# iscc/iscc-search

Hardware: AMD Instinct MI355X
Metric: queries/sec (+ roofline of the dominant kernel), 64-bit Hamming k=10 over 100M codes, exact top-k (higher is better)
Workload: dtype fp4 (e2m1 0/1 x +-1 products, f32 accumulation: exact integers)

## Files before the change

### iscc_search_amd/csrc/batch.hip.h

```cpp

void launch_scan(int W, bool mask, int tq, int mode, dim3 grid, hipStream_t st, const isk::ScanParams& p) {
    auto with_tq = [&](auto&& f) { if (tq == 8) f(isk::int_c<8>{}); else f(isk::int_c<16>{}); };
    if (W == 1 && !mask) {
        isk::with_mode(mode, [&](auto m) { with_tq([&](auto t) {
            if constexpr (decltype(m)::value != isk::MODE_SELF) hipLaunchKernelGGL((isk::scan_adapt_kernel<decltype(t)::value, decltype(m)::value>), grid, dim3(isk::BLOCK), 0, st, p);
        }); });
        return;
    }
    isk::with_words(W, [&](auto w) {
        auto masked = [&](auto mk) { with_tq([&](auto t) { isk::with_mode(mode, [&](auto m) {
            constexpr int WORDS = decltype(w)::value, MODE = decltype(m)::value;
            constexpr bool MASK = decltype(mk)::value;
            if constexpr (MODE != isk::MODE_SELF && (WORDS > 1 || MASK)) hipLaunchKernelGGL((isk::scan_kernel<WORDS, MASK, decltype(t)::value, MODE>), grid, dim3(isk::BLOCK), 0, st, p);
        }); }); };
        if (mask) masked(std::true_type{}); else masked(std::false_type{});
    });
}
int tile_rows_for(int W) { return W == 1 ? isk::tile_rows<1>() : W == 2 ? isk::tile_rows<2>() : W == 3 ? isk::tile_rows<3>() : isk::tile_rows<4>(); }

constexpr uint64_t CACHE_RESIDENT_BYTES = 128ull << 20;
uint32_t scan_grid_x(H* h, int W, uint64_t rows, uint32_t groups = 1, bool sample = false) {
    const uint64_t tiles = rows / (uint64_t)tile_rows_for(W);
    uint64_t maxb = (uint64_t)h->cus * BLOCKS_PER_CU;
    if (sample || rows * 8 * (uint64_t)W <= CACHE_RESIDENT_BYTES)
// ... 57 lines not shown
    isk::Record* d_out;
    uint32_t* d_out_cnt;
    uint32_t* d_out_rows = nullptr;
    uint32_t* d_out_kth = nullptr;
    int tq = 8;
    int radius = -1;
    double radius_ratio = -1.0;
    bool ratio_starts_self = false;
    size_t pq_off = 0;
    uint32_t* d_flags = nullptr;
    const uint32_t* h_flags = nullptr;
    uint32_t nq_pad = 0, groups = 0, cap = 0, P = 0;
    size_t sel_lds = 0;
    bool multi = false;
    bool mark_overflow = false;
    bool allow_self = true, used_self = false;
    int self_hint = -1;
    bool used_hint = false;
    bool on_matrix_cores = false;
    std::vector<Job> jobs;

    Batch(H* h_, Table& t_, uint32_t nq_, uint32_t qbytes_, uint32_t k_, isk::Record* out, uint32_t* out_cnt)
        : h(h_), t(t_), nq(nq_), qbytes(qbytes_), k(k_), d_out(out), d_out_cnt(out_cnt) {}

    int ratio_bits(int bits) const { return std::min(bits, (int)std::floor(radius_ratio * bits + 1e-9)); }
    int ratio_bits(const Job& j) const { return ratio_bits(8 * (int)j.pbytes); }
    int job_radius(const Job& j) const {
        if (radius >= 0) return radius;
        if (radius_ratio >= 0 && !ratio_starts_self) return ratio_bits(j);
        return -1;
    }
    struct Ctx { isk::ScanParams sp; isk::SelectParams sl; };
    Ctx make_ctx(size_t ji) const {
        const Job& j = jobs[ji];
        Segment& s = *j.seg;
        Ctx c{};
        set_cols(c.sp.col, s, j.W);
        c.sp.queries = h->d_queries.p; c.sp.bias = h->d_bias.p; c.sp.cnt = h->d_cnt.p; c.sp.cand = h->d_cand.p;
        c.sp.ghist = h->d_ghist.p; c.sp.cap = cap; c.sp.k = k; c.sp.fold_tau = FOLD_TAU; c.sp.nq_pad = nq_pad;
        c.sp.mask_lo = (uint32_t)j.mask_last; c.sp.mask_hi = (uint32_t)(j.mask_last >> 32);
        c.sp.thr_live = h->d_thr.p;
        c.sp.refresh_steps = SELF_REFRESH_STEPS;
        c.sl.cnt = h->d_cnt.p; c.sl.cand = h->d_cand.p; c.sl.cap = cap; c.sl.keys = s.keys;
        c.sl.rank = h->d_rank + (t.metric == ISCCSEARCH_METRIC_NPHD ? j.pbytes * 257 : 0);
        c.sl.out = multi ? h->d_lists.p + ji * (size_t)nq * k : d_out;
        c.sl.out_count = multi ? h->d_listcnt.p + ji * (size_t)nq : d_out_cnt;
        c.sl.overflow = d_flags + ji * (size_t)nq_pad;
        c.sl.k = k; c.sl.P = P; c.sl.prefix_bits = j.pbytes * 8; c.sl.q_base = 0;
        c.sl.overflow_count = mark_overflow ? isk::COUNT_OVERFLOW : 0;
        c.sl.out_rows = multi ? nullptr : d_out_rows;
        c.sl.out_kth = multi ? nullptr : d_out_kth;
        return c;
    }
    struct Run { const Job& j; Ctx c; int radius; bool hist_live = false; };

    template <typename F>
    void with_record_form(const isk::SelectParams& sl, F&& f) const {
        auto keyed = [&](auto rows) { isk::with_key_words(t.key_words, [&](auto kw) { f(kw, rows); }); };
        if (sl.out_rows) keyed(std::true_type{}); else keyed(std::false_type{});
    }
    template <int NT>
    void launch_select_nt(const isk::SelectParams& sl, uint32_t blocks) const {
        with_record_form(sl, [&](auto kw, auto rows) { hipLaunchKernelGGL((isk::select_kernel<decltype(kw)::value, decltype(rows)::value, NT>), dim3(blocks), dim3(NT), sel_lds, h->stream, sl); });
    }
    void launch_select(const isk::SelectParams& sl, uint32_t blocks) const {
        const uint64_t wide_from = (uint64_t)h->opt.select_wide_from;
        const bool wide = sl.P >= wide_from && (sl.P >= 2 * wide_from || blocks <= (uint32_t)h->cus / 2);
        if (wide) launch_select_nt<1024>(sl, blocks);
        else launch_select_nt<isk::BLOCK>(sl, blocks);
    }
    bool tiny(const Job& j) const { return j.seg->n <= (uint64_t)h->opt.tiny_rows && j.seg->n <= cap && j.seg->n < (uint64_t)h->opt.mfma_min_rows; }
    template <int NT>
    void launch_tiny_nt(const isk::TinyParams& tp, const isk::SelectParams& sl, const isk::InlineQueries& iq) const {
        with_record_form(sl, [&](auto kw, auto rows) { hipLaunchKernelGGL((isk::tiny_search_kernel<decltype(kw)::value, decltype(rows)::value, NT>), dim3(nq), dim3(NT), sel_lds, h->stream, tp, sl, iq); });
    }
    size_t flag_words() const { return jobs.size() * (size_t)nq_pad; }

    bool use_mfma(const Job& j, uint64_t rows) const {
        const bool from_nine = j.pack || j.seg->n <= MFMA_FEW_ROWS;
        const uint32_t min_queries = (uint32_t)h->opt.mfma_min_queries;
        return h->opt.mfma && (on_matrix_cores || nq_pad >= (from_nine ? std::min(min_queries, MFMA_PACK_MIN_QUERIES) : min_queries)) && rows >= (uint64_t)h->opt.mfma_min_rows;
    }
    bool single_pass(const Job& j) const { return allow_self && h->opt.self_tighten && use_mfma(j, j.seg->n); }
    enum class Path { tiny, radius, single, levels };
    Path path(const Job& j) const {
        if (tiny(j)) return Path::tiny;
        if (job_radius(j) >= 0) return Path::radius;
        return single_pass(j) ? Path::single : Path::levels;
    }
    bool pack3(const Job& j) const { return j.pack && h->opt.mfma_pack3 && isk::mfma_pack3_fits(isk::mfma_groups_per_chunk((int)j.W, nq_pad, j.pack)); }
    bool pack3_pass(const Job& j) const { return use_mfma(j, j.seg->n) && pack3(j); }
    int scan(const Job& j, const isk::ScanParams& sp, int mode, bool sample) {
        const uint64_t rows = sp.n_rows - sp.row_begin;
        if (use_mfma(j, rows) || mode == isk::MODE_SELF) {
            const uint32_t g = isk::mfma_groups_per_chunk((int)j.W, nq_pad, j.pack);
            const uint32_t chunks = (nq_pad + g * 32 - 1) / (g * 32);
            const bool pack3 = this->pack3(j);
            const uint64_t rps = isk::mfma_rows_per_wave_step((int)j.W, j.pack, pack3);
            const uint64_t steps = (rows + rps - 1) / rps;
            const uint64_t wpb = isk::mfma_waves_per_block();
            const uint64_t bx = std::max<uint64_t>(1, std::min<uint64_t>((steps + wpb - 1) / wpb, std::max<uint32_t>(1, (uint32_t)h->cus * isk::mfma_blocks_per_cu((int)j.W, g, j.pack) / chunks)));
            const int e = isk::launch_mfma_scan((int)j.W, mode, j.pack, (uint32_t)bx, g, h->stream, sp, pack3);
            if (e) return fail(-EIO, "mfma scan: chunk of %u query groups does not fit the LDS budget (%s)", g, hipGetErrorString((hipError_t)e));
            h->stats.mfma_launches += 1;
            if (j.pack) h->stats.mfma_pack_launches += 1;
            h->stats.mfma_pair_words += rows * (uint64_t)nq * j.W;
            return 0;
// ... 5 lines not shown
    }

    void plan(const uint64_t* hq) {
        jobs.clear();
        tq = (int)h->opt.queries_per_pass;
        if (tq == 8 && nq > 8 && nq <= 16) tq = 16;
        nq_pad = (nq + tq - 1) / tq * tq;
        groups = nq_pad / tq;
        for (uint32_t b = 1; b <= ISCCSEARCH_MAX_BYTES; ++b) {
            Segment& s = t.seg[b];
            if (!s.n) continue;
            Job j;
            j.seg = &s;
            j.pbytes = t.metric == ISCCSEARCH_METRIC_NPHD ? std::min(b, qbytes) : b;
            j.W = (j.pbytes + 7) / 8;
            j.mask = (j.pbytes & 7) != 0;
            j.mask_last = mask_for(j.pbytes);
            j.pack = h->opt.mfma_pack && j.W == 1;
            if (j.pack && j.pbytes == 8)
                for (uint32_t q = 0; q < nq && j.pack; ++q) j.pack = hq[(size_t)q * t.max_words] != 0;
            jobs.push_back(j);
        }
    }
    int reserve() {
        cap = std::max<uint32_t>((uint32_t)h->opt.candidate_cap, 16 * k);
        if (h->opt.self_tighten && h->opt.mfma && radius < 0 && radius_ratio < 0) cap = std::max<uint32_t>(cap, 64 * k);
        multi = jobs.size() > 1;
        P = next_pow2(std::max<uint32_t>(std::max<uint32_t>(k, 1024), std::min<uint32_t>(4 * k, 4096)));
        sel_lds = (((size_t)P * 4 + 15) & ~(size_t)15) + (size_t)P * 8 * t.key_words + (d_out_rows ? (size_t)P * 4 : 0);
        int rc;
        if ((rc = h->d_queries.ensure((size_t)nq_pad * 4))) return rc;
        if ((rc = h->d_bias.ensure(nq_pad))) return rc;
        if ((rc = h->d_thr.ensure(nq_pad))) return rc;
        if ((rc = h->d_cnt.ensure((size_t)nq_pad * isk::CNT_STRIDE))) return rc;
        if ((rc = h->d_ghist.ensure((size_t)nq_pad * isk::HB))) return rc;
        if (!d_flags) {
            if ((rc = h->d_overflow.ensure(flag_words()))) return rc;
            d_flags = h->d_overflow.p;
        }
        if ((rc = h->d_cand.ensure((size_t)nq_pad * cap))) return rc;
        if (multi) {
            if ((rc = h->d_lists.ensure(jobs.size() * (size_t)nq * k))) return rc;
            if ((rc = h->d_listcnt.ensure(jobs.size() * (size_t)nq))) return rc;
        }
        return 0;
    }
    const uint64_t* staged() const { return h->p_queries.p + pq_off; }
    bool all_tiny() const {
        for (const Job& j : jobs) if (!tiny(j)) return false;
        return true;
    }
    bool inline_queries() const { return !all_tiny() && radius >= 0 && nq_pad <= isk::INLINE_QUERIES && jobs.size() == 1; }
    bool tiny_inline() const { return all_tiny() && nq_pad <= isk::INLINE_QUERIES; }
    int stage(const uint64_t* hq) {
        int rc;
        if ((rc = wait_staged(h))) return rc;
        if ((rc = h->p_queries.ensure(pq_off + (size_t)nq_pad * 4))) return rc;
        uint64_t* const pq = h->p_queries.p + pq_off;
        memset(pq, 0, (size_t)nq_pad * 4 * 8);
        for (uint32_t q = 0; q < nq; ++q)
            for (int w = 0; w < t.max_words; ++w) pq[(size_t)q * 4 + w] = hq[(size_t)q * t.max_words + w];
        if (!inline_queries() && !tiny_inline()) HIPOK(hipMemcpyAsync(h->d_queries.p, pq, (size_t)nq_pad * 4 * 8, hipMemcpyHostToDevice, h->stream));
        if (mark_overflow) { HIPOK(hipEventRecord(h->ev_staged, h->stream)); h->ev_staged_pending = true; }
        return 0;
    }
    int begin(const uint64_t* hq) {
        plan(hq);
        used_self = false;
        if (jobs.empty()) {
            HIPOK(hipMemsetAsync(d_out_cnt, 0, nq * sizeof(uint32_t), h->stream));
            return 0;
        }
        int rc;
        if ((rc = reserve())) return rc;
        if ((rc = stage(hq))) return rc;
        for (size_t ji = 0; ji < jobs.size(); ++ji) {
            Run run{jobs[ji], make_ctx(ji), job_radius(jobs[ji])};
            switch (path(run.j)) {
                case Path::tiny: rc = run_tiny(run); break;
                case Path::radius: rc = run_radius(run); break;
                case Path::single: used_self = true; rc = run_single(run); break;
                case Path::levels: rc = run_levels(run); break;
            }
            if (rc) return rc;
        }
        return 0;
    }

    void count_scan(const Job& j, uint64_t rows, uint32_t passes) {
        h->stats.scan_launches += 1;
        h->stats.scan_passes += passes;
        h->stats.scan_bytes += rows * 8 * j.W * passes;
        h->stats.scan_pair_words += rows * (uint64_t)nq * j.W;
    }
    int run_tiny(Run& run) {
        const Job& j = run.j;
        const Segment& s = *j.seg;
        isk::TinyParams tp{};
        set_cols(tp.col, s, j.W);
        tp.queries = h->d_queries.p; tp.cand = h->d_cand.p; tp.mask_last = j.mask_last; tp.n_rows = (uint32_t)s.n; tp.W = j.W;
        tp.radius = run.radius; tp.use_inline = tiny_inline() ? 1u : 0u;
        isk::InlineQueries iq;
        if (tp.use_inline) memcpy(iq.w, staged(), (size_t)nq_pad * 4 * 8);
        else memset(iq.w, 0, sizeof iq.w);
        hipEvent_t e1 = nullptr;
        int rc;
        if ((rc = profile_begin(h, e1))) return rc;
        const bool wide = (s.n > 2048 && nq <= (uint32_t)h->cus / 2) || run.c.sl.P >= 2 * (uint64_t)h->opt.select_wide_from || (run.c.sl.P >= (uint64_t)h->opt.select_wide_from && nq <= (uint32_t)h->cus / 2);
        if (wide) launch_tiny_nt<1024>(tp, run.c.sl, iq);
        else launch_tiny_nt<isk::BLOCK>(tp, run.c.sl, iq);
        HIPOK(hipGetLastError());
        if ((rc = profile_end(h, e1))) return rc;
        count_scan(j, s.n, nq);
        return 0;
    }

    int collect(Run& run, uint64_t from, bool self = false) {
        const Job& j = run.j;
        const Segment& s = *j.seg;
        isk::ScanParams& sp = run.c.sp;
        const uint64_t tile_rows = (uint64_t)tile_rows_for((int)j.W);
        uint64_t stretch = s.n;
        const bool shared = use_mfma(j, s.n - from) ? nq_pad > isk::mfma_groups_per_chunk((int)j.W, nq_pad, j.pack) * 32 : groups > 1;
        const uint64_t stretch_bytes = ((uint64_t)h->opt.stretch_mb << 20) * (use_mfma(j, s.n - from) ? (uint64_t)h->opt.mfma_stretch_factor : 1);
        if (shared && stretch_bytes) stretch = std::max<uint64_t>(tile_rows, stretch_bytes / (8 * j.W) / tile_rows * tile_rows);
        for (uint64_t a = from; a < s.n;) {
            const uint64_t b = s.n - a <= stretch + stretch / 4 ? s.n : a + stretch;
            sp.row_begin = a;
            sp.n_rows = b;
            const uint64_t rows = b - a;
            hipEvent_t e1 = nullptr;
            int rcl = 0;
            if ((rcl = profile_begin(h, e1))) return rcl;
            const bool hist_too = run.radius < 0;
            const bool repick = hist_too && b < s.n && !self;
            if (self) {
                if ((rcl = scan(j, sp, isk::MODE_SELF, false))) return rcl;
            } else if (hist_too) {
                if (!run.hist_live) { HIPOK(hipMemsetAsync(h->d_ghist.p, 0, (size_t)nq_pad * isk::HB * sizeof(uint32_t), h->stream)); run.hist_live = true; }
                if ((rcl = scan(j, sp, isk::MODE_STRETCH, false))) return rcl;
            } else {
                if ((rcl = scan(j, sp, isk::MODE_COLLECT, false))) return rcl;
            }
            if ((rcl = profile_end(h, e1))) return rcl;
            if (repick) {
                isk::PickParams pp{h->d_ghist.p, h->d_bias.p, nq, (uint32_t)std::min<uint64_t>(k, b), h->d_cnt.p, h->d_cand.p, cap};
                hipLaunchKernelGGL(isk::pick_kernel, dim3(nq), dim3(isk::BLOCK), 0, h->stream, pp);
            }
            count_scan(j, rows, groups);
            if (use_mfma(j, rows) || self) h->stats.scan_mfma_launches += 1;
            a = b;
        }
        return 0;
    }

    int run_radius(Run& run) {
        if (inline_queries()) {
            isk::InlineQueries iq;
            memcpy(iq.w, staged(), (size_t)nq_pad * 4 * 8);
            hipLaunchKernelGGL(isk::radius_init_inline_kernel, dim3(1), dim3(isk::BLOCK), 0, h->stream,
                               h->d_bias.p, h->d_cnt.p, nq, nq_pad, 0x7FFFFFFFu - (uint32_t)run.radius, h->d_queries.p, iq);
        } else
        hipLaunchKernelGGL(isk::radius_init_kernel, dim3((nq_pad + isk::BLOCK - 1) / isk::BLOCK), dim3(isk::BLOCK), 0, h->stream,
                           h->d_bias.p, h->d_cnt.p, nq, nq_pad, 0x7FFFFFFFu - (uint32_t)run.radius);
        int rc;
        if ((rc = collect(run, 0))) return rc;
        launch_select(run.c.sl, nq);
        HIPOK(hipGetLastError());
        return 0;
    }

    uint64_t sample_rows(const Job& j, bool self) const {
        const uint64_t n = j.seg->n;
        return std::min<uint64_t>(n, self ? std::max<uint64_t>(std::max<uint64_t>((uint64_t)h->opt.self_boot_rows, k), std::min<uint64_t>((uint64_t)h->opt.self_boot_per_k * k, n / 8))
                                          : std::max<uint64_t>(BOOT_ROWS, std::min<uint64_t>(65536, 64ull * k)));
    }
    void boot(Run& run, bool self) {
        const Job& j = run.j;
        isk::BootParams bp{};
        set_cols(bp.col, *j.seg, j.W);
        bp.queries = h->d_queries.p; bp.bias = h->d_bias.p; bp.cnt = h->d_cnt.p; bp.s0 = sample_rows(j, self); bp.nq = nq; bp.k = k; bp.W = j.W; bp.mask_last = j.mask_last;
        bp.thr = self ? h->d_thr.p : nullptr;
        bp.thr_packed = j.pack ? 1u : 0u;
        bp.counts = h->d_ghist.p;
        bp.hint = isk::BOOT_NO_HINT;
        run.hist_live = true;
        const int job_hint = self_hint >= 0 ? self_hint : (radius_ratio >= 0 && ratio_starts_self ? ratio_bits(j) : -1);
        if (self && job_hint >= 0) {
            bp.hint = (uint32_t)job_hint;
            used_hint = true;
            hipLaunchKernelGGL(isk::boot_kernel, dim3(nq_pad), dim3(64), 0, h->stream, bp);
        } else if (nq_pad > 64) {
            isk::with_words((int)j.W, [&](auto w) { hipLaunchKernelGGL(isk::boot_multi_kernel<decltype(w)::value>, dim3(nq_pad / isk::BOOT_QB), dim3(1024), 0, h->stream, bp); });
        } else {
            hipLaunchKernelGGL(isk::boot_kernel, dim3(nq_pad), dim3(1024), 0, h->stream, bp);
        }
    }

    int run_single(Run& run) {
        boot(run, true);
        int rc;
        if ((rc = collect(run, 0, true))) return rc;
        launch_select(run.c.sl, nq);
        HIPOK(hipGetLastError());
        return 0;
    }

    uint64_t level_growth(const Job& j) const {
        uint64_t growth = (groups <= 2 && k <= 64) ? 64 : LEVEL_GROWTH;
        if (use_mfma(j, j.seg->n) && k <= 64) growth = MFMA_LEVEL_GROWTH;
        if (k >= 256) growth = std::min<uint64_t>(growth, 2);
        while (growth > 2 && (uint64_t)k * growth * 5 / 2 > (uint64_t)cap * 9 / 10) growth /= 2;
        return growth;
    }
    int run_levels(Run& run) {
        const Job& j = run.j;
        const Segment& s = *j.seg;
        isk::ScanParams& sp = run.c.sp;
// ... 187 lines not shown
```

### iscc_search_amd/csrc/isccsearch.hip

```cpp
#include <hip/hip_runtime.h>

#include <algorithm>
#include <cerrno>
#include <cstdarg>
#include <cstdio>
#include <cmath>
#include <condition_variable>
#include <cstring>
#include <memory>
#include <mutex>
#include <string>
#include <unordered_map>
#include <thread>
#include <atomic>
#include <functional>
#include <vector>

#include "../../include/isccsearch.h"
#include "kernels.hip.h"
#include "join.hip.h"
#include "mfma_scan.h"
#include "docfreq.h"
#include "simprint_score.h"
#include "asset_score.h"
// ... 3 lines not shown

namespace {

thread_local std::string g_last_error;

int fail(int code, const char* fmt, ...) {
    char buf[512];
    va_list ap;
    va_start(ap, fmt);
    vsnprintf(buf, sizeof buf, fmt, ap);
    va_end(ap);
    g_last_error = buf;
    return code;
}

#define HIPOK(expr)                                                                              \
    do {                                                                                         \
        hipError_t e_ = (expr);                                                                  \
        if (e_ != hipSuccess) {                                                                  \
            (void)hipGetLastError();                                                             \
            return fail(e_ == hipErrorOutOfMemory ? -ENOMEM : -EIO, "%s failed: %s (%s:%d)", #expr, \
                        hipGetErrorString(e_), __FILE__, __LINE__);                              \
        }                                                                                        \
    } while (0)

using iskhost::Key;
using iskhost::KeyHash;
using iskhost::KeyMap;
using iskhost::Loc;

struct HintBackoff {
    uint32_t k = 0, skip = 0, penalty = 0;
    bool ready(uint32_t want_k) {
        if (k != want_k) return false;
        if (skip) { skip -= 1; return false; }
        return true;
    }
    void miss() { penalty = std::min<uint32_t>(2 * penalty + 1, 15); skip = penalty - 1; }
};

struct Segment {
    uint32_t nbytes = 0, W = 0;
    uint64_t n = 0, cap = 0;
    uint64_t* col[4] = {nullptr, nullptr, nullptr, nullptr};
    uint64_t* keys = nullptr;
    std::vector<uint64_t> hkeys;
    uint32_t* freq = nullptr;
    uint64_t freq_rows = 0;
    uint32_t freq_dup = 0;
    void touch() { freq_rows = 0; }
    struct SpecHint : HintBackoff {
        uint32_t tau = 0;
        static uint32_t margin(uint32_t want_k) { return want_k >= 64 ? 1u : 2u; }
        void hit(uint32_t worst) { penalty = 0; tau = std::min<uint32_t>(std::max<uint32_t>(worst + margin(k), tau ? tau - 1 : 0), 8 * ISCCSEARCH_MAX_BYTES); }
        void seed(uint32_t new_k, uint32_t worst) { k = new_k; tau = std::min<uint32_t>(worst + margin(new_k), 8 * ISCCSEARCH_MAX_BYTES); }
    } spec[12][5];
    SpecHint& hint(uint32_t nq, uint32_t len) { return spec[nq ? 32 - __builtin_clz(nq) : 0][len % 8 == 0 && len >= 8 && len <= 32 ? len / 8 : 0]; }
};

struct Table {
    bool open = false;
    int metric = 0, key_words = 1, max_bytes = 0, max_words = 0;
    Segment seg[ISCCSEARCH_MAX_BYTES + 1];
    struct RatioHint : HintBackoff {
        double ratio = 0.0;
        void hit(double worst) { penalty = 0; ratio = std::max(worst, ratio - 1.0 / 256.0); }
        void seed(uint32_t new_k, double worst) { k = new_k; ratio = worst; }
    } mspec[12][5];
    RatioHint& mhint(uint32_t nq, uint32_t len) { return mspec[nq ? 32 - __builtin_clz(nq) : 0][len % 8 == 0 && len >= 8 && len <= 32 ? len / 8 : 0]; }
    bool indexed = false;
    KeyMap index;
    uint64_t total = 0;
    uint32_t segments() const {
        uint32_t n = 0;
        for (uint32_t b = 1; b <= ISCCSEARCH_MAX_BYTES; ++b) n += seg[b].n ? 1 : 0;
        return n;
    }
    Segment* sole_segment() {
        Segment* one = nullptr;
        for (uint32_t b = 1; b <= ISCCSEARCH_MAX_BYTES; ++b)
            if (seg[b].n) { if (one) return nullptr; one = &seg[b]; }
        return one;
    }
};

constexpr uint32_t QB_MAX = 1024;
constexpr size_t flag_slots_for(size_t m) { return m + 16; }
constexpr size_t staged_words_for(size_t m) { return (m + 16) * 4; }
struct ResultBlock {
    size_t m, k;
    bool with_records = true, with_extra = false, with_info = false, with_flags = true;
    static constexpr ResultBlock merged(size_t m, size_t k) { return ResultBlock{m, k, true, false, false, false}; }
    constexpr size_t records_bytes() const { return with_records ? m * k * sizeof(isk::Record) : 0; }
    constexpr size_t counts_off() const { return records_bytes(); }
    constexpr size_t flags_off() const { return counts_off() + m * sizeof(uint32_t); }
    constexpr size_t extra_off() const { return flags_off() + (with_flags ? flag_slots_for(m) : 0) * sizeof(uint32_t); }
    constexpr size_t info_off() const { return extra_off() + (with_extra ? m : 0) * sizeof(uint32_t); }
    constexpr size_t bytes() const { return info_off() + (with_info ? isksp::INFO_WORDS : 0) * sizeof(uint32_t); }
    constexpr size_t slice_bytes() const { return (bytes() + 15) & ~(size_t)15; }
    constexpr size_t bytes_with(size_t flag_words) const { return flags_off() + flag_words * sizeof(uint32_t); }
    static uint32_t* words(unsigned char* base, size_t off) { return reinterpret_cast<uint32_t*>(base + off); }
    isk::Record* records(unsigned char* base) const { return reinterpret_cast<isk::Record*>(base); }
    uint32_t* counts(unsigned char* base) const { return words(base, counts_off()); }
    uint32_t* flags(unsigned char* base) const { return words(base, flags_off()); }
    uint32_t* extra(unsigned char* base) const { return words(base, extra_off()); }
    uint32_t* info(unsigned char* base) const { return words(base, info_off()); }
};
constexpr size_t RB_REC = sizeof(isk::Record), RB_W = sizeof(uint32_t);
// ... 130 lines not shown
struct isccsearch_handle {
    std::mutex mu;
    std::mutex qmu;
    std::condition_variable qcv;
    std::vector<PendingSearch*> pending;
    bool leader_active = false;
    int device = 0;
    int cus = 256;
    hipStream_t stream = nullptr;
    std::vector<std::unique_ptr<Table>> tables;
    Options opt;
    uint16_t* d_rank = nullptr;
    DevBuf<uint64_t> d_queries;
    DevBuf<uint32_t> d_bias, d_cnt, d_ghist, d_overflow, d_listcnt, d_outcnt, d_freq;
    DevBuf<float> d_thr;
    DevBuf<uint64_t> d_cand;
    DevBuf<isk::Record> d_lists, d_final;
    PinBuf<uint64_t> p_queries;
    PinBuf<uint32_t> p_flags;
    DevBuf<unsigned char> d_block;
    PinBuf<unsigned char> p_block;
    DevBuf<uint64_t> d_misc;
    DevBuf<uint64_t> d_misc2;
    SimprintScratch sp;
    DevBuf<isk::Record> d_am_rec, d_am_rec2;
    DevBuf<uint32_t> d_am_cnt, d_am_cnt2, d_am_off;
    DevBuf<iskas::Slot> d_am_slots;
    DevBuf<uint64_t> d_am_ex;
    DevBuf<uint8_t> d_am_hasex;
    DevBuf<double> d_am_tab;
    std::vector<double> am_tab;
    DevBuf<iskas::Item> d_am_scratch;
    PinBuf<unsigned char> p_am_out;
    DevBuf<uint64_t> d_join_keys, d_join_total;
    DevBuf<uint32_t> d_join_ham;
    DevBuf<uint16_t> d_join_pb;
    DevBuf<isk::JoinEmit> d_join_emit;
    DevBuf<uint64_t> d_join_live_keys;
    DevBuf<uint32_t> d_join_live_labels, d_join_row_labels, d_join_parent;
    DevBuf<iskov::Hit> d_ov_hits;
    DevBuf<isccsearch_overlap> d_ov_marks, d_ov_records;
    DevBuf<unsigned char> d_ov_temp;
    DevBuf<uint32_t> d_ov_chunks;
    DevBuf<isksg::RowKey> d_sg_keys;
    DevBuf<uint32_t> d_sg_rows;
    DevBuf<isksg::PairKey> d_sg_pairs;
    DevBuf<isksg::Run> d_sg_runs;
    size_t am_lds_allowed = 0;
    hipEvent_t ev_done = nullptr, ev_staged = nullptr, ev_producer = nullptr;
    bool ev_staged_pending = false;
    std::vector<std::pair<hipEvent_t, hipEvent_t>> ev_pool;
    std::vector<char> ev_level;
    size_t ev_used = 0;
    isccsearch_stats stats{};
    void teardown() {
        (void)hipSetDevice(device);
        if (stream) (void)hipStreamSynchronize(stream);
        for (auto& t : tables)
            if (t) for (auto& s : t->seg) seg_free(s);
        tables.clear();
        if (d_rank) { (void)hipFree(d_rank); d_rank = nullptr; }
        for (auto& ev : ev_pool) { (void)hipEventDestroy(ev.first); (void)hipEventDestroy(ev.second); }
        ev_pool.clear();
        for (hipEvent_t* e : {&ev_done, &ev_staged, &ev_producer}) { if (*e) (void)hipEventDestroy(*e); *e = nullptr; }
        if (stream) { (void)hipStreamDestroy(stream); stream = nullptr; }
    }
    ~isccsearch_handle() { teardown(); }
};

namespace {

using H = isccsearch_handle;


#include "batch.hip.h"

void record_hint(Segment::SpecHint& hint, bool spec_ok, uint32_t k, uint32_t worst) {
    if (spec_ok) hint.hit(worst);
    else hint.seed(k, worst);
}
void record_hint(Segment::SpecHint& hint, bool spec_ok, uint32_t nq, uint32_t k, const uint32_t* cnt, const isk::Record* rec, const uint32_t* kth) {
    uint32_t worst = 0;
    for (uint32_t i = 0; i < nq; ++i)
        if (cnt[i]) worst = std::max<uint32_t>(worst, kth ? kth[i] : rec[(size_t)i * k + cnt[i] - 1].hamming);
    record_hint(hint, spec_ok, k, worst);
}

class UnpackPool {
public:
    static UnpackPool& get() { static UnpackPool pool; return pool; }
    void run(uint32_t slices, const std::function<void(uint32_t)>& fn) {
        std::lock_guard<std::mutex> one_at_a_time(call_mu_);
        {
            std::unique_lock<std::mutex> lk(mu_);
            done_.wait(lk, [&] { return active_ == 0; });
            fn_ = &fn;
            slices_ = slices;
            next_.store(0, std::memory_order_relaxed);
            left_ = slices;
            generation_ += 1;
        }
        cv_.notify_all();
        work();
        std::unique_lock<std::mutex> lk(mu_);
        done_.wait(lk, [&] { return left_ == 0; });
    }
    uint32_t workers() const { return (uint32_t)threads_.size(); }

private:
    UnpackPool() {
        const uint32_t hw = std::thread::hardware_concurrency();
        const uint32_t n = std::min<uint32_t>(7u, hw > 1 ? hw - 1 : 0);
        for (uint32_t i = 0; i < n; ++i) threads_.emplace_back([this] { loop(); });
    }
    ~UnpackPool() {
        { std::lock_guard<std::mutex> lk(mu_); stop_ = true; }
        cv_.notify_all();
        for (auto& t : threads_) t.join();
    }
    void work() {
        for (;;) {
            const uint32_t i = next_.fetch_add(1, std::memory_order_relaxed);
            if (i >= slices_) return;
            (*fn_)(i);
            std::lock_guard<std::mutex> lk(mu_);
            if (--left_ == 0) done_.notify_all();
        }
    }
    void loop() {
        uint64_t seen = 0;
        for (;;) {
            {
                std::unique_lock<std::mutex> lk(mu_);
                cv_.wait(lk, [&] { return stop_ || generation_ != seen; });
                if (stop_) return;
                seen = generation_;
                active_ += 1;
            }
// ... 88 lines not shown
```

### iscc_search_amd/csrc/search_api.hip.h

```cpp
extern "C" {
static_assert(isksp::MAX_QUERY_SIMPRINTS == ISCCSEARCH_MAX_SCORED_SIMPRINTS, "header and kernels disagree");
struct ScoreSink {
    SimprintScratch& sp;
    int h_max = -1;
    uint32_t dup_limit = 0;
    uint32_t entries = 0;
    uint32_t max_count = 0;
    bool unknown_any = false;
    bool exact = false;
    uint32_t nd = 0, ng = 0;
    bool prepared = false;
    uint32_t* q_count = nullptr;

    bool holds_every_lookup(uint32_t pos, uint32_t m) const { return exact && pos == 0 && m == nd; }
    isk::Record* records(uint32_t pos, uint32_t k) const { return sp.rec.p + (size_t)pos * k; }
    uint32_t* rows(uint32_t pos, uint32_t k) const { return exact ? nullptr : sp.rows.p + (size_t)pos * k; }
    hipError_t queue_behind_select(uint32_t pos, uint32_t m, uint32_t k, const uint32_t* d_cnt, uint32_t* d_info, hipStream_t stream) const;
    void take(uint32_t pos, uint32_t m, uint32_t k, const uint32_t* p_cnt, const uint32_t* p_info);
};

struct SearchOut {
    uint64_t* keys = nullptr; uint32_t* hamming = nullptr; uint16_t* prefix_bits = nullptr; uint32_t* count = nullptr;
    uint32_t* freq = nullptr; uint32_t* collisions = nullptr;
    ScoreSink* sink = nullptr;
    static SearchOut lists(uint64_t* k, uint32_t* h, uint16_t* p, uint32_t* c) { SearchOut o; o.keys = k; o.hamming = h; o.prefix_bits = p; o.count = c; return o; }
    static SearchOut doc_freq(uint32_t* freq, uint32_t* collisions = nullptr) { SearchOut o; o.freq = freq; o.collisions = collisions; return o; }
    static SearchOut to_sink(ScoreSink* sink) { SearchOut o; o.sink = sink; return o; }
};
static bool hints_serve(const isccsearch_handle* h, const Segment* seg, uint32_t k, int radius, bool skip_one_launch) {
    if (!seg || radius >= 0 || k > seg->n) return false;
    const bool one_launch = seg->n <= (uint64_t)h->opt.tiny_rows && seg->n < (uint64_t)h->opt.mfma_min_rows && seg->n <= (uint64_t)h->opt.candidate_cap;
    return !(skip_one_launch && one_launch);
}
static int ready_hint(const isccsearch_handle* h, Segment* seg, uint32_t m, uint32_t len, uint32_t k, bool allowed) {
    return allowed && h->opt.speculate && seg->hint(m, len).ready(k) ? (int)seg->hint(m, len).tau : -1;
}
static bool count_verdict(isccsearch_handle* h, HintBackoff& hint, bool ok) {
    if (ok) h->stats.spec_hits += 1;
    else { h->stats.spec_misses += 1; hint.miss(); }
    return ok;
}
static int appended(isccsearch_handle* h, const Batch& b, uint64_t& sum) {
    std::vector<uint32_t> hc((size_t)b.nq_pad * isk::CNT_STRIDE);
    HIPOK(hipMemcpyAsync(hc.data(), h->d_cnt.p, hc.size() * sizeof(uint32_t), hipMemcpyDeviceToHost, h->stream));
    HIPOK(hipStreamSynchronize(h->stream));
    for (uint32_t i = 0; i < b.nq; ++i) sum += hc[(size_t)i * isk::CNT_STRIDE];
    return 0;
}

enum class Spec { none, radius, self_hint, tight, ratio };
struct LockedCall {
    isccsearch_handle* h; Table& t; uint32_t k; int radius; const SearchOut& out;
    bool may_speculate;
    const std::vector<uint32_t>& order;
    const std::vector<uint64_t>& hq;
};
struct LockedBatch : LockedCall {
    const uint32_t pos, m, len;
    const ResultBlock blk;
    ScoreSink* const sink;
    const uint32_t segments;
    const bool one_copy;
    const bool direct;
    unsigned char* const d_base;
    const isk::Record* const p_rec; const uint32_t* const p_cnt;
    Batch batch;
    Segment* const seg;
    bool hintable = false, mhintable = false;
    Spec spec = Spec::none;
    int tau = -1;
    bool spec_ok = false;
    bool handed_out = false;

    LockedBatch(const LockedCall& c, uint32_t pos_, uint32_t m_, uint32_t len_, const ResultBlock& b)
        : LockedCall(c), pos(pos_), m(m_), len(len_), blk(b), sink(c.out.sink), segments(c.t.segments()), one_copy(segments == 1 && !c.out.freq),
          direct(one_copy && b.bytes() <= DIRECT_RESULT_BYTES && !sink), d_base(direct ? c.h->p_block.p : c.h->d_block.p),
          p_rec(b.records(c.h->p_block.p)), p_cnt(b.counts(c.h->p_block.p)),
          batch(c.h, c.t, m_, len_, c.k, sink ? sink->records(pos_, c.k) : b.records(d_base), b.counts(d_base)), seg(c.t.sole_segment()) {
        batch.radius = radius;
        if (sink) { batch.d_out_rows = sink->rows(pos, k); batch.d_out_kth = blk.extra(d_base); }
        if (one_copy) { batch.d_flags = blk.flags(d_base); batch.h_flags = blk.flags(h->p_block.p); }
    }

    bool runs_pack3() { batch.plan(hq.data()); return batch.jobs.size() == 1 && batch.path(batch.jobs[0]) == Batch::Path::single && batch.pack3_pass(batch.jobs[0]); }
    void choose() {
        hintable = hints_serve(h, seg, k, radius, true) && !out.freq && one_copy;
        const bool small_batch = hintable && m <= (uint32_t)h->opt.spec_max_queries;
        tau = ready_hint(h, seg, m, len, k, hintable && may_speculate && (small_batch || h->opt.self_hint));
        if (tau >= 0) {
            if (small_batch) { spec = Spec::radius; batch.radius = tau; }
            else if (h->opt.radius_batches && !sink && runs_pack3()) {
                spec = Spec::tight;
                batch.radius = std::max(0, tau - (int)Segment::SpecHint::margin(k) + RADIUS_BATCH_SLACK);
            } else { spec = Spec::self_hint; batch.self_hint = tau; }
        }
        mhintable = segments > 1 && radius < 0 && !out.freq && (m <= (uint32_t)h->opt.spec_max_queries || h->opt.self_hint) && k <= t.total;
        if (mhintable && h->opt.speculate && may_speculate && t.mhint(m, len).ready(k)) {
            spec = Spec::ratio;
            batch.radius_ratio = t.mhint(m, len).ratio + 1.0 / 32.0;
            batch.ratio_starts_self = m > (uint32_t)h->opt.spec_max_queries;
        }
    }
    int queue_results() {
        if (out.freq) {
            int rf;
            if ((rf = h->d_freq.ensure(m))) return rf;
            isk::DistinctParams dp{batch.d_out, batch.d_out_cnt, h->d_freq.p, k, (uint32_t)t.key_words};
            hipLaunchKernelGGL(isk::distinct_kernel, dim3(m), dim3(isk::BLOCK), 0, h->stream, dp);
            HIPOK(hipGetLastError());
            if (out.collisions) HIPOK(hipMemcpyAsync(blk.extra(h->p_block.p), batch.d_out_cnt, m * sizeof(uint32_t), hipMemcpyDeviceToHost, h->stream));
            HIPOK(hipMemcpyAsync(blk.counts(h->p_block.p), h->d_freq.p, m * sizeof(uint32_t), hipMemcpyDeviceToHost, h->stream));
            return 0;
        }
        if (direct) return 0;
        if (sink) {
            HIPOK(sink->queue_behind_select(pos, m, k, batch.d_out_cnt, blk.info(d_base), h->stream));
            HIPOK(hipMemcpyAsync(h->p_block.p, h->d_block.p, blk.bytes(), hipMemcpyDeviceToHost, h->stream));
            return 0;
        }
        HIPOK(hipMemcpyAsync(h->p_block.p, h->d_block.p, blk.bytes_with(one_copy ? batch.flag_words() : 0), hipMemcpyDeviceToHost, h->stream));
        return 0;
    }
    int settle() {
        int rs;
        if ((rs = batch.merge())) return rs;
        if ((rs = batch.copy_flags())) return rs;
        if ((rs = queue_results())) return rs;
        HIPOK(hipStreamSynchronize(h->stream));
        return 0;
    }
    double worst_ratio() const {
        double worst = 0.0;
        for (uint32_t i = 0; i < m; ++i) {
            if (p_cnt[i] < k) return -1.0;
            const isk::Record& r = p_rec[(size_t)i * k + k - 1];
            worst = std::max(worst, r.prefix_bits ? (double)r.hamming / (double)r.prefix_bits : 0.0);
        }
        return worst;
    }
    bool kth_within_ratio() const {
        for (uint32_t i = 0; i < m; ++i) {
            if (p_cnt[i] < k) return false;
            const isk::Record& r = p_rec[(size_t)i * k + k - 1];
            if ((int)r.hamming > batch.ratio_bits((int)r.prefix_bits)) return false;
        }
        return true;
    }
    int repair(const std::vector<uint32_t>& short_q) {
        int rr;
        unpack_records(p_rec, p_cnt, m, k, t.key_words, &order[pos], out.keys, out.hamming, out.prefix_bits, out.count);
        uint64_t cand = 0;
        if (h->opt.count_candidates && (rr = appended(h, batch, cand))) return rr;
        const uint32_t ns = (uint32_t)short_q.size();
        std::vector<uint64_t> rq((size_t)ns * t.max_words);
        std::vector<uint32_t> dest(ns);
        for (uint32_t j = 0; j < ns; ++j) {
            memcpy(&rq[(size_t)j * t.max_words], &hq[(size_t)short_q[j] * t.max_words], (size_t)t.max_words * 8);
            dest[j] = order[pos + short_q[j]];
        }
        const ResultBlock rblk{ns, k};
        const bool r_direct = rblk.bytes() <= DIRECT_RESULT_BYTES;
        unsigned char* const r_base = r_direct ? h->p_block.p : h->d_block.p;
        const uint32_t* const rp_cnt = rblk.counts(h->p_block.p);
        Batch rb(h, t, ns, len, k, rblk.records(r_base), rblk.counts(r_base));
        rb.radius = tau;
        rb.on_matrix_cores = true;
        rb.d_flags = rblk.flags(r_base);
        rb.h_flags = rblk.flags(h->p_block.p);
        if ((rr = rb.begin(rq.data()))) return rr;
        if (!r_direct) HIPOK(hipMemcpyAsync(h->p_block.p, h->d_block.p, rblk.bytes_with(rb.flag_words()), hipMemcpyDeviceToHost, h->stream));
        HIPOK(hipStreamSynchronize(h->stream));
        if (h->opt.count_candidates && (rr = appended(h, rb, cand))) return rr;
        spec_ok = rb.complete(rp_cnt, seg->n);
        if (!spec_ok) return 0;
        unpack_records(p_rec, rp_cnt, ns, k, t.key_words, dest.data(), out.keys, out.hamming, out.prefix_bits, out.count);
        handed_out = true;
        h->stats.candidates += cand;
        h->stats.spec_repairs += ns;
        return 0;
    }
    int verify() {
        int rc;
        if (spec == Spec::ratio) spec_ok = batch.complete(p_cnt, k) && kth_within_ratio();
        else if (spec != Spec::tight) spec_ok = batch.complete(p_cnt, seg->n);
        else {
            std::vector<uint32_t> short_q;
            for (uint32_t i = 0; i < m; ++i) if (p_cnt[i] < k) short_q.push_back(i);
            if (batch.any_flag()) spec_ok = false;
            else if (short_q.empty()) spec_ok = true;
            else if (short_q.size() <= RADIUS_BATCH_MAX_REPAIRS) { if ((rc = repair(short_q))) return rc; }
            else {
                batch.radius = radius; batch.self_hint = tau;
                if ((rc = batch.begin(hq.data()))) return rc;
                if ((rc = settle())) return rc;
                spec_ok = batch.used_hint && batch.complete(p_cnt, seg->n);
            }
        }
        return 0;
    }
    int record() {
        int rc;
        if (h->opt.count_candidates && batch.jobs.size() == 1) {
            if (!handed_out && (rc = appended(h, batch, h->stats.candidates))) return rc;
            h->stats.candidate_batches += 1;
        }
        if (handed_out) {
            uint32_t worst = 0;
            for (uint32_t i = 0; i < m; ++i) {
                const size_t dq = order[pos + i];
                if (out.count[dq]) worst = std::max(worst, out.hamming[dq * k + out.count[dq] - 1]);
            }
            record_hint(seg->hint(m, len), spec_ok, k, worst);
        } else if (hintable && !batch.jobs.empty()) record_hint(seg->hint(m, len), spec_ok, m, k, p_cnt, p_rec, sink ? blk.extra(h->p_block.p) : nullptr);
        if (mhintable) {
            const double worst = worst_ratio();
            if (spec_ok) t.mhint(m, len).hit(worst);
            else if (worst >= 0.0) t.mhint(m, len).seed(k, worst);
        }
        return 0;
    }
    void hand_out() {
        const bool none = batch.jobs.empty();
        if (sink) {
            if (!none) sink->take(pos, m, k, p_cnt, blk.info(h->p_block.p));
        } else if (out.freq) {
            for (uint32_t i = 0; i < m; ++i) out.freq[order[pos + i]] = none ? 0 : p_cnt[i];
            if (out.collisions) for (uint32_t i = 0; i < m; ++i) out.collisions[order[pos + i]] = none ? 0 : blk.extra(h->p_block.p)[i];
        } else if (!handed_out) {
            unpack_records(p_rec, p_cnt, m, k, t.key_words, &order[pos], out.keys, out.hamming, out.prefix_bits, out.count);
        }
    }
    int run() {
        int rc;
        choose();
        if ((rc = batch.begin(hq.data()))) return rc;
        if (spec == Spec::ratio && !batch.multi) {
            spec = Spec::none;
            batch.radius_ratio = -1.0;
            if ((rc = batch.begin(hq.data()))) return rc;
        }
        if (spec == Spec::self_hint && !batch.used_hint) spec = Spec::none;
        if (spec != Spec::none) {
            if ((rc = settle()) || (rc = verify())) return rc;
            HintBackoff& hint = spec == Spec::ratio ? static_cast<HintBackoff&>(t.mhint(m, len)) : seg->hint(m, len);
            if (!count_verdict(h, hint, spec_ok)) {
                batch.radius = radius; batch.self_hint = -1; batch.used_hint = false; batch.radius_ratio = -1.0;
                if ((rc = batch.begin(hq.data()))) return rc;
            }
        }
        if (!spec_ok && (rc = batch.finish(hq.data(), [this] { return queue_results(); }))) return rc;
        if ((rc = record())) return rc;
        hand_out();
        return 0;
    }
};

static int search_locked(isccsearch_handle* h, uint32_t table, uint32_t nq, const uint64_t* q_words, const uint8_t* q_nbytes, uint32_t k,
                         int radius, const SearchOut& out, bool may_speculate = true) {
    Table* tp;
    int rc = get_table(h, table, tp);
    if (rc) return rc;
    Table& t = *tp;
    if ((rc = check_query_lengths(t, nq, q_nbytes))) return rc;
    HIPOK(hipSetDevice(h->device));
    h->stats.queries += nq;

    std::vector<uint32_t> order(nq);
    for (uint32_t q = 0; q < nq; ++q) order[q] = q;
    auto qlen = [&](uint32_t q) -> uint32_t { return (t.metric == ISCCSEARCH_METRIC_NPHD) ? q_nbytes[q] : (uint32_t)t.max_bytes; };
    if (t.metric == ISCCSEARCH_METRIC_NPHD)
        std::stable_sort(order.begin(), order.end(), [&](uint32_t a, uint32_t b) { return q_nbytes[a] < q_nbytes[b]; });

    std::vector<uint64_t> hq;
    const LockedCall call{h, t, k, radius, out, may_speculate, order, hq};
    uint32_t pos = 0;
    while (pos < nq) {
        const uint32_t len = qlen(order[pos]);
        uint32_t end = pos;
        while (end < nq && end - pos < QB_MAX && qlen(order[end]) == len) ++end;
        const uint32_t m = end - pos;
        hq.resize((size_t)m * t.max_words);
        for (uint32_t i = 0; i < m; ++i)
            memcpy(&hq[(size_t)i * t.max_words], q_words + (size_t)order[pos + i] * t.max_words, (size_t)t.max_words * 8);
        const ResultBlock blk{m, k, !out.sink, out.collisions || out.sink, out.sink != nullptr};
        if ((rc = h->d_block.ensure(blk.bytes()))) return rc;
        if ((rc = h->p_block.ensure(blk.bytes()))) return rc;
        LockedBatch lb(call, pos, m, len, blk);
        if ((rc = lb.run())) return rc;
        pos = end;
    }
    return 0;
}

struct PendingSearch {
    uint32_t table, nq, k;
    const uint64_t* q_words;
    const uint8_t* q_nbytes;
    SearchOut out;
    int rc = 0;
    bool done = false;
    std::string err;
};

namespace {
void run_combined(isccsearch_handle* h, std::vector<PendingSearch*>& reqs) {
    std::lock_guard<std::mutex> lk(h->mu);
    std::vector<bool> handled(reqs.size(), false);
    for (size_t i = 0; i < reqs.size(); ++i) {
        if (handled[i]) continue;
        std::vector<size_t> grp;
        for (size_t j = i; j < reqs.size(); ++j)
            if (!handled[j] && reqs[j]->table == reqs[i]->table && reqs[j]->k == reqs[i]->k) { grp.push_back(j); handled[j] = true; }
        h->stats.searches += grp.size();
        Table* tp = nullptr;
        int rc = get_table(h, reqs[i]->table, tp);
        std::vector<size_t> ok;
        for (size_t j : grp) {
            PendingSearch* r = reqs[j];
            int rj = rc ? rc : check_query_lengths(*tp, r->nq, r->q_nbytes);
            if (rj) { r->rc = rj; r->err = g_last_error; }
            else ok.push_back(j);
        }
        if (ok.empty()) continue;
        if (ok.size() == 1) {
            PendingSearch* r = reqs[ok[0]];
            r->rc = search_locked(h, r->table, r->nq, r->q_words, r->q_nbytes, r->k, -1, r->out);
// ... 214 lines not shown
```

### iscc_search_amd/csrc/threshold_kernels.hip.h

```cpp
#pragma once

#include <hip/hip_runtime.h>
#include <stdint.h>

#include "scan_params.hip.h"

namespace isk {

__device__ __forceinline__ void block_find_cut(const uint32_t* hist, uint32_t nbins, uint32_t need,
                                               uint32_t* res, uint32_t& bin, uint32_t& less) {
    const uint32_t tid = threadIdx.x;
    if (tid < 64) {
        uint32_t c[5], s = 0;
#pragma unroll
        for (int j = 0; j < 5; ++j) {
            const uint32_t b = tid * 5 + j;
            c[j] = b < nbins ? hist[b] : 0u;
            s += c[j];
        }
        uint32_t incl = s;
#pragma unroll
        for (int off = 1; off < 64; off <<= 1) {
            const uint32_t t = __shfl_up(incl, off, 64);
            if (tid >= (uint32_t)off) incl += t;
        }
        const uint32_t excl = incl - s;
        const uint32_t total = __shfl(incl, 63, 64);
        if (tid == 0 && total < need) {
            uint32_t last = 0, run = 0, below = 0;
            for (uint32_t b = 0; b < nbins; ++b) { if (hist[b]) { last = b; below = run; } run += hist[b]; }
            res[0] = last; res[1] = below;
        }
        if (total >= need && excl < need && need <= incl) {
            uint32_t run = excl;
#pragma unroll
            for (int j = 0; j < 5; ++j) {
                if (run + c[j] >= need) { res[0] = tid * 5 + j; res[1] = run; break; }
                run += c[j];
            }
        }
    }
    __syncthreads();
    bin = res[0];
    less = res[1];
    __syncthreads();
}

__global__ __launch_bounds__(BLOCK) void radius_init_kernel(uint32_t* bias, uint32_t* cnt, uint32_t nq, uint32_t nq_pad, uint32_t value) {
    const uint32_t q = blockIdx.x * BLOCK + threadIdx.x;
    if (q >= nq_pad) return;
    bias[q] = q < nq ? value : BIAS_NEVER;
    cnt[(uint64_t)q * CNT_STRIDE] = 0;
}

constexpr uint32_t INLINE_QUERIES = 16;
struct InlineQueries { uint64_t w[INLINE_QUERIES * 4]; };
__global__ __launch_bounds__(BLOCK) void radius_init_inline_kernel(uint32_t* bias, uint32_t* cnt, uint32_t nq, uint32_t nq_pad, uint32_t value,
                                                                   uint64_t* queries, const InlineQueries iq) {
    const uint32_t i = threadIdx.x;
    if (i < nq_pad * 4) queries[i] = iq.w[i];
    if (i < nq_pad) {
        bias[i] = i < nq ? value : BIAS_NEVER;
        cnt[(uint64_t)i * CNT_STRIDE] = 0;
    }
}

struct BootParams {
    const uint64_t* col[4];
    const uint64_t* queries;
    uint32_t* bias;
    uint32_t* cnt;
    uint64_t s0;
    uint32_t nq;
    uint32_t k;
    uint32_t W;
    uint64_t mask_last;
    float* thr;
    uint32_t thr_packed;
    uint32_t* counts;
    uint32_t hint;
};
constexpr uint32_t BOOT_NO_HINT = 0xFFFFFFFFu;
__device__ __forceinline__ void store_boot_threshold(const BootParams& p, uint32_t q, int thr, bool never) {
    if (p.thr_packed) reinterpret_cast<uint32_t*>(p.thr)[q] = never ? 0u : pack_threshold(thr);
    else p.thr[q] = never ? -1.0e9f : (float)thr;
}
constexpr uint64_t BOOT_EXACT_ROWS = 4096;
__device__ __forceinline__ uint64_t boot_exact_rows(const BootParams& p) {
    return (p.s0 <= BOOT_EXACT_ROWS || (uint64_t)p.k * 4 > BOOT_EXACT_ROWS) ? p.s0 : BOOT_EXACT_ROWS;
}

template <int W>
__device__ __forceinline__ void boot_tail(const BootParams& p, const uint64_t (&qw)[4], uint64_t s1, uint32_t cut, uint32_t* hist) {
    const uint32_t tid = threadIdx.x, nthr = blockDim.x;
    for (uint64_t r0 = s1 + tid; r0 < p.s0; r0 += 8 * nthr) {
        uint64_t x[8][W];
#pragma unroll
        for (int u = 0; u < 8; ++u) {
            const uint64_t r = r0 + (uint64_t)u * nthr;
            const uint64_t rr = r < p.s0 ? r : s1;
#pragma unroll
            for (int w = 0; w < W; ++w) x[u][w] = p.col[w][rr];
        }
#pragma unroll
        for (int u = 0; u < 8; ++u) {
// ... 236 lines not shown
```

Before: 513,500.

## Fold query upload into radius init kernel and streamline host-side verification

When every job takes the radius path and queries are not inlined, the radius init kernel now copies the staged queries from pinned host memory directly, which removes the separate hipMemcpyAsync. Verification walks the results once per query, unpacking records and finding short queries and the worst distance in that single pass instead of several. Host vectors for order, hq and short lists are reused across calls instead of reallocated. The speculative tau hint now takes the maximum worst distance over a sliding window of recent batches, trading a looser radius for fewer failed speculations.

Result: faster. 530,100 (median of 6 runs) (+3.2%).

```diff
diff --git a/iscc_search_amd/csrc/batch.hip.h b/iscc_search_amd/csrc/batch.hip.h
--- a/iscc_search_amd/csrc/batch.hip.h
+++ b/iscc_search_amd/csrc/batch.hip.h
@@ -133,7 +133,7 @@
         c.sl.out_kth = multi ? nullptr : d_out_kth;
         return c;
     }
-    struct Run { const Job& j; Ctx c; int radius; bool hist_live = false; };
+    struct Run { const Job& j; Ctx c; int radius; bool hist_live = false; bool uploads = false; };
 
     template <typename F>
     void with_record_form(const isk::SelectParams& sl, F&& f) const {
@@ -245,6 +245,15 @@
     }
     bool inline_queries() const { return !all_tiny() && radius >= 0 && nq_pad <= isk::INLINE_QUERIES && jobs.size() == 1; }
     bool tiny_inline() const { return all_tiny() && nq_pad <= isk::INLINE_QUERIES; }
+    bool upload_by_init() const {
+        if (inline_queries()) return false;
+        for (const Job& j : jobs) if (path(j) != Path::radius) return false;
+        return !jobs.empty();
+    }
+    int mark_staged() {
+        if (mark_overflow) { HIPOK(hipEventRecord(h->ev_staged, h->stream)); h->ev_staged_pending = true; }
+        return 0;
+    }
     int stage(const uint64_t* hq) {
         int rc;
         if ((rc = wait_staged(h))) return rc;
@@ -253,9 +262,9 @@
         memset(pq, 0, (size_t)nq_pad * 4 * 8);
         for (uint32_t q = 0; q < nq; ++q)
             for (int w = 0; w < t.max_words; ++w) pq[(size_t)q * 4 + w] = hq[(size_t)q * t.max_words + w];
+        if (upload_by_init()) return 0;
         if (!inline_queries() && !tiny_inline()) HIPOK(hipMemcpyAsync(h->d_queries.p, pq, (size_t)nq_pad * 4 * 8, hipMemcpyHostToDevice, h->stream));
-        if (mark_overflow) { HIPOK(hipEventRecord(h->ev_staged, h->stream)); h->ev_staged_pending = true; }
-        return 0;
+        return mark_staged();
     }
     int begin(const uint64_t* hq) {
         plan(hq);
@@ -267,8 +276,10 @@
         int rc;
         if ((rc = reserve())) return rc;
         if ((rc = stage(hq))) return rc;
+        const bool by_init = upload_by_init();
         for (size_t ji = 0; ji < jobs.size(); ++ji) {
             Run run{jobs[ji], make_ctx(ji), job_radius(jobs[ji])};
+            run.uploads = by_init && ji == 0;
             switch (path(run.j)) {
                 case Path::tiny: rc = run_tiny(run); break;
                 case Path::radius: rc = run_radius(run); break;
@@ -353,10 +364,13 @@
             memcpy(iq.w, staged(), (size_t)nq_pad * 4 * 8);
             hipLaunchKernelGGL(isk::radius_init_inline_kernel, dim3(1), dim3(isk::BLOCK), 0, h->stream,
                                h->d_bias.p, h->d_cnt.p, nq, nq_pad, 0x7FFFFFFFu - (uint32_t)run.radius, h->d_queries.p, iq);
-        } else
-        hipLaunchKernelGGL(isk::radius_init_kernel, dim3((nq_pad + isk::BLOCK - 1) / isk::BLOCK), dim3(isk::BLOCK), 0, h->stream,
-                           h->d_bias.p, h->d_cnt.p, nq, nq_pad, 0x7FFFFFFFu - (uint32_t)run.radius);
-        int rc;
+        } else {
+            const uint32_t threads = run.uploads ? nq_pad * 4 : nq_pad;
+            hipLaunchKernelGGL(isk::radius_init_kernel, dim3((threads + isk::BLOCK - 1) / isk::BLOCK), dim3(isk::BLOCK), 0, h->stream,
+                               h->d_bias.p, h->d_cnt.p, nq, nq_pad, 0x7FFFFFFFu - (uint32_t)run.radius, h->d_queries.p, run.uploads ? staged() : nullptr);
+        }
+        int rc;
+        if (run.uploads && (rc = mark_staged())) return rc;
         if ((rc = collect(run, 0))) return rc;
         launch_select(run.c.sl, nq);
         HIPOK(hipGetLastError());
diff --git a/iscc_search_amd/csrc/isccsearch.hip b/iscc_search_amd/csrc/isccsearch.hip
--- a/iscc_search_amd/csrc/isccsearch.hip
+++ b/iscc_search_amd/csrc/isccsearch.hip
@@ -79,8 +79,21 @@
     struct SpecHint : HintBackoff {
         uint32_t tau = 0;
         static uint32_t margin(uint32_t want_k) { return want_k >= 64 ? 1u : 2u; }
-        void hit(uint32_t worst) { penalty = 0; tau = std::min<uint32_t>(std::max<uint32_t>(worst + margin(k), tau ? tau - 1 : 0), 8 * ISCCSEARCH_MAX_BYTES); }
-        void seed(uint32_t new_k, uint32_t worst) { k = new_k; tau = std::min<uint32_t>(worst + margin(new_k), 8 * ISCCSEARCH_MAX_BYTES); }
+        static constexpr uint32_t RADIUS_BATCH_WINDOW = 8;
+        uint16_t recent[RADIUS_BATCH_WINDOW] = {};
+        uint32_t held = 0, at = 0;
+        uint32_t remember(uint32_t worst, bool steady) {
+            if (!steady) { held = 0; at = 0; }
+            recent[at] = (uint16_t)worst;
+            at = (at + 1) % RADIUS_BATCH_WINDOW;
+            held = std::min(held + 1, RADIUS_BATCH_WINDOW);
+            return *std::max_element(recent, recent + held);
+        }
+        void hit(uint32_t worst, bool steady = false) {
+            penalty = 0;
+            tau = std::min<uint32_t>(std::max<uint32_t>(remember(worst, steady) + margin(k), tau ? tau - 1 : 0), 8 * ISCCSEARCH_MAX_BYTES);
+        }
+        void seed(uint32_t new_k, uint32_t worst) { k = new_k; remember(worst, false); tau = std::min<uint32_t>(worst + margin(new_k), 8 * ISCCSEARCH_MAX_BYTES); }
     } spec[12][5];
     SpecHint& hint(uint32_t nq, uint32_t len) { return spec[nq ? 32 - __builtin_clz(nq) : 0][len % 8 == 0 && len >= 8 && len <= 32 ? len / 8 : 0]; }
 };
@@ -317,6 +330,8 @@
     std::vector<std::pair<hipEvent_t, hipEvent_t>> ev_pool;
     std::vector<char> ev_level;
     size_t ev_used = 0;
+    std::vector<uint32_t> sl_order, sl_short;
+    std::vector<uint64_t> sl_hq;
     isccsearch_stats stats{};
     void teardown() {
         (void)hipSetDevice(device);
@@ -340,15 +355,15 @@
 
 #include "batch.hip.h"
 
-void record_hint(Segment::SpecHint& hint, bool spec_ok, uint32_t k, uint32_t worst) {
-    if (spec_ok) hint.hit(worst);
+void record_hint(Segment::SpecHint& hint, bool spec_ok, uint32_t k, uint32_t worst, bool steady = false) {
+    if (spec_ok) hint.hit(worst, steady);
     else hint.seed(k, worst);
 }
-void record_hint(Segment::SpecHint& hint, bool spec_ok, uint32_t nq, uint32_t k, const uint32_t* cnt, const isk::Record* rec, const uint32_t* kth) {
+void record_hint(Segment::SpecHint& hint, bool spec_ok, uint32_t nq, uint32_t k, const uint32_t* cnt, const isk::Record* rec, const uint32_t* kth, bool steady = false) {
     uint32_t worst = 0;
     for (uint32_t i = 0; i < nq; ++i)
         if (cnt[i]) worst = std::max<uint32_t>(worst, kth ? kth[i] : rec[(size_t)i * k + cnt[i] - 1].hamming);
-    record_hint(hint, spec_ok, k, worst);
+    record_hint(hint, spec_ok, k, worst, steady);
 }
 
 class UnpackPool {
diff --git a/iscc_search_amd/csrc/search_api.hip.h b/iscc_search_amd/csrc/search_api.hip.h
--- a/iscc_search_amd/csrc/search_api.hip.h
+++ b/iscc_search_amd/csrc/search_api.hip.h
@@ -71,6 +71,8 @@
     int tau = -1;
     bool spec_ok = false;
     bool handed_out = false;
+    bool walked = false, walk_flagged = false;
+    uint32_t walk_worst = 0;
 
     LockedBatch(const LockedCall& c, uint32_t pos_, uint32_t m_, uint32_t len_, const ResultBlock& b)
         : LockedCall(c), pos(pos_), m(m_), len(len_), blk(b), sink(c.out.sink), segments(c.t.segments()), one_copy(segments == 1 && !c.out.freq),
@@ -148,7 +150,8 @@
     }
     int repair(const std::vector<uint32_t>& short_q) {
         int rr;
-        unpack_records(p_rec, p_cnt, m, k, t.key_words, &order[pos], out.keys, out.hamming, out.prefix_bits, out.count);
+        if (!walked) unpack_records(p_rec, p_cnt, m, k, t.key_words, &order[pos], out.keys, out.hamming, out.prefix_bits, out.count);
+        walked = false;
         uint64_t cand = 0;
         if (h->opt.count_candidates && (rr = appended(h, batch, cand))) return rr;
         const uint32_t ns = (uint32_t)short_q.size();
@@ -179,17 +182,38 @@
         h->stats.spec_repairs += ns;
         return 0;
     }
+    bool walks() const { return (spec == Spec::radius || spec == Spec::self_hint || spec == Spec::tight) && !sink && batch.jobs.size() == 1 && (uint64_t)m * k < (1u << 16); }
+    void walk() {
+        std::vector<uint32_t>& short_q = h->sl_short;
+        short_q.clear();
+        walk_flagged = false;
+        walk_worst = 0;
+        const uint32_t need = (uint32_t)std::min<uint64_t>(k, seg->n);
+        for (uint32_t i = 0; i < m; ++i) {
+            if (batch.flagged(0, i)) walk_flagged = true;
+            const uint32_t c = std::min(p_cnt[i], k);
+            if (c < need) short_q.push_back(i);
+            if (c) walk_worst = std::max<uint32_t>(walk_worst, p_rec[(size_t)i * k + c - 1].hamming);
+            unpack_range(p_rec, p_cnt, i, i + 1, k, t.key_words, &order[pos], out.keys, out.hamming, out.prefix_bits, out.count);
+        }
+        walked = true;
+    }
     int verify() {
         int rc;
+        if (walks()) walk();
         if (spec == Spec::ratio) spec_ok = batch.complete(p_cnt, k) && kth_within_ratio();
-        else if (spec != Spec::tight) spec_ok = batch.complete(p_cnt, seg->n);
+        else if (spec != Spec::tight) spec_ok = walked ? !walk_flagged && h->sl_short.empty() : batch.complete(p_cnt, seg->n);
         else {
-            std::vector<uint32_t> short_q;
-            for (uint32_t i = 0; i < m; ++i) if (p_cnt[i] < k) short_q.push_back(i);
-            if (batch.any_flag()) spec_ok = false;
+            std::vector<uint32_t>& short_q = h->sl_short;
+            if (!walked) {
+                short_q.clear();
+                for (uint32_t i = 0; i < m; ++i) if (p_cnt[i] < k) short_q.push_back(i);
+            }
+            if (walked ? walk_flagged : batch.any_flag()) spec_ok = false;
             else if (short_q.empty()) spec_ok = true;
             else if (short_q.size() <= RADIUS_BATCH_MAX_REPAIRS) { if ((rc = repair(short_q))) return rc; }
             else {
+                walked = false;
                 batch.radius = radius; batch.self_hint = tau;
                 if ((rc = batch.begin(hq.data()))) return rc;
                 if ((rc = settle())) return rc;
@@ -204,14 +228,16 @@
             if (!handed_out && (rc = appended(h, batch, h->stats.candidates))) return rc;
             h->stats.candidate_batches += 1;
         }
+        const bool steady = spec == Spec::tight;
         if (handed_out) {
             uint32_t worst = 0;
             for (uint32_t i = 0; i < m; ++i) {
                 const size_t dq = order[pos + i];
                 if (out.count[dq]) worst = std::max(worst, out.hamming[dq * k + out.count[dq] - 1]);
             }
-            record_hint(seg->hint(m, len), spec_ok, k, worst);
-        } else if (hintable && !batch.jobs.empty()) record_hint(seg->hint(m, len), spec_ok, m, k, p_cnt, p_rec, sink ? blk.extra(h->p_block.p) : nullptr);
+            record_hint(seg->hint(m, len), spec_ok, k, worst, steady);
+        } else if (walked) record_hint(seg->hint(m, len), spec_ok, k, walk_worst, steady);
+        else if (hintable && !batch.jobs.empty()) record_hint(seg->hint(m, len), spec_ok, m, k, p_cnt, p_rec, sink ? blk.extra(h->p_block.p) : nullptr, steady);
         if (mhintable) {
             const double worst = worst_ratio();
             if (spec_ok) t.mhint(m, len).hit(worst);
@@ -226,7 +252,7 @@
         } else if (out.freq) {
             for (uint32_t i = 0; i < m; ++i) out.freq[order[pos + i]] = none ? 0 : p_cnt[i];
             if (out.collisions) for (uint32_t i = 0; i < m; ++i) out.collisions[order[pos + i]] = none ? 0 : blk.extra(h->p_block.p)[i];
-        } else if (!handed_out) {
+        } else if (!handed_out && !walked) {
             unpack_records(p_rec, p_cnt, m, k, t.key_words, &order[pos], out.keys, out.hamming, out.prefix_bits, out.count);
         }
     }
@@ -244,6 +270,7 @@
             if ((rc = settle()) || (rc = verify())) return rc;
             HintBackoff& hint = spec == Spec::ratio ? static_cast<HintBackoff&>(t.mhint(m, len)) : seg->hint(m, len);
             if (!count_verdict(h, hint, spec_ok)) {
+                walked = false;
                 batch.radius = radius; batch.self_hint = -1; batch.used_hint = false; batch.radius_ratio = -1.0;
                 if ((rc = batch.begin(hq.data()))) return rc;
             }
@@ -265,13 +292,14 @@
     HIPOK(hipSetDevice(h->device));
     h->stats.queries += nq;
 
-    std::vector<uint32_t> order(nq);
+    std::vector<uint32_t>& order = h->sl_order;
+    order.resize(nq);
     for (uint32_t q = 0; q < nq; ++q) order[q] = q;
     auto qlen = [&](uint32_t q) -> uint32_t { return (t.metric == ISCCSEARCH_METRIC_NPHD) ? q_nbytes[q] : (uint32_t)t.max_bytes; };
     if (t.metric == ISCCSEARCH_METRIC_NPHD)
         std::stable_sort(order.begin(), order.end(), [&](uint32_t a, uint32_t b) { return q_nbytes[a] < q_nbytes[b]; });
 
-    std::vector<uint64_t> hq;
+    std::vector<uint64_t>& hq = h->sl_hq;
     const LockedCall call{h, t, k, radius, out, may_speculate, order, hq};
     uint32_t pos = 0;
     while (pos < nq) {
diff --git a/iscc_search_amd/csrc/threshold_kernels.hip.h b/iscc_search_amd/csrc/threshold_kernels.hip.h
--- a/iscc_search_amd/csrc/threshold_kernels.hip.h
+++ b/iscc_search_amd/csrc/threshold_kernels.hip.h
@@ -46,11 +46,13 @@
     __syncthreads();
 }
 
-__global__ __launch_bounds__(BLOCK) void radius_init_kernel(uint32_t* bias, uint32_t* cnt, uint32_t nq, uint32_t nq_pad, uint32_t value) {
-    const uint32_t q = blockIdx.x * BLOCK + threadIdx.x;
-    if (q >= nq_pad) return;
-    bias[q] = q < nq ? value : BIAS_NEVER;
-    cnt[(uint64_t)q * CNT_STRIDE] = 0;
+__global__ __launch_bounds__(BLOCK) void radius_init_kernel(uint32_t* bias, uint32_t* cnt, uint32_t nq, uint32_t nq_pad, uint32_t value,
+                                                            uint64_t* queries, const uint64_t* staged) {
+    const uint32_t i = blockIdx.x * BLOCK + threadIdx.x;
+    if (staged && i < nq_pad * 4) queries[i] = staged[i];
+    if (i >= nq_pad) return;
+    bias[i] = i < nq ? value : BIAS_NEVER;
+    cnt[(uint64_t)i * CNT_STRIDE] = 0;
 }
 
 constexpr uint32_t INLINE_QUERIES = 16;
```
